# greysun/GraphEmbeddings

Measured on AMD Instinct MI355X. Metric: scored triples/sec/GPU (d=200), higher is better.
Workload: dtype f32

## Files before the change

graphembeddings_amd/build.py:

```python
from __future__ import annotations

import os
import shutil
import subprocess
import sys

HERE = os.path.dirname(os.path.abspath(__file__))
CSRC = os.path.join(HERE, "csrc")
LIB = os.path.join(HERE, "libge_hip.so")
SOURCES = ["ge_capi.hip", "ge_complex.hip", "ge_rows.hip", "ge_hole.hip", "ge_1vk.hip", "ge_train.hip", "ge_prep_big.hip", "ge_shard.hip", "ge_spectral.hip", "ge_rank.hip", "ge_rank_pipe.hip", "ge_rank_f16.hip", "ge_known.hip", "ge_transx.hip", "ge_transr.hip", "ge_transx_rank.hip", "ge_neighbors.hip", "ge_transx_relrank.hip", "ge_classify.hip"]
HEADERS = ["ge_common.h", "ge_launch.h", "ge_step_id.h", "ge_prep.h", "ge_complex_dev.h", "ge_rank_dev.h", "ge_sweep_route.h", "ge_trans.h", "ge_trans_dev.h", "ge_f16_dev.h", "ge_topk_dev.h", "ge_bernoulli_dev.h", os.path.join("..", "..", "include", "ge_hip.h")]
ARCH = "gfx950"


def _hipcc() -> str:
    for cand in (os.environ.get("HIPCC"), shutil.which("hipcc"), "/opt/rocm/bin/hipcc"):
        if cand and os.path.exists(cand):
            return cand
    raise RuntimeError("hipcc not found: libge_hip.so cannot be built (ROCm toolchain required)")


def needs_build() -> bool:
    if not os.path.exists(LIB):
        return True
    t = os.path.getmtime(LIB)
    deps = [os.path.join(CSRC, s) for s in SOURCES + HEADERS] + [os.path.abspath(__file__)]
    return any(os.path.getmtime(p) > t for p in deps)


FILE_FLAGS = {"ge_hole.hip": ["-fno-slp-vectorize"]}
OBJDIR = os.path.join(HERE, "_obj")


def build(force: bool = False, verbose: bool = False, extra_flags=()) -> str:
    if not force and not needs_build():
        return LIB
    os.makedirs(OBJDIR, exist_ok=True)
    cc = _hipcc()
    common = ["-O3", f"--offload-arch={ARCH}", "-std=c++17", "-fPIC", "-Wall", "-Wno-unused-function", *extra_flags,
              *os.environ.get("GE_CXXFLAGS", "").split()]
    procs = []
    for src in SOURCES:
        obj = os.path.join(OBJDIR, src.replace(".hip", ".o"))
        cmd = [cc, *common, *FILE_FLAGS.get(src, []), "-c", src, "-o", obj]
# ... 19 lines not shown
```

graphembeddings_amd/csrc/ge_complex.hip:

```cpp
#include "ge_complex_dev.h"
#include "ge_launch.h"

namespace ge {

template <bool SPEC, int VEC, int LPT, int NITER>
__global__ __launch_bounds__(kBlock) void complex_score_kernel(
    const float* __restrict__ table, int64_t N, int d, const int32_t* __restrict__ triples, int64_t B,
    float max_norm, int apply_sigmoid, float* __restrict__ out, float label, float l2,
    const float* __restrict__ table_sumsq, int64_t ld) {
  constexpr int GPW = kWave / LPT;
  const int lane = threadIdx.x & (kWave - 1), sub = lane % LPT, grp = lane / LPT;
  const int64_t wave = ((int64_t)blockIdx.x * blockDim.x + threadIdx.x) >> 6;
  const int64_t nwaves = ((int64_t)gridDim.x * blockDim.x) >> 6;
  const int k = d >> 1, nvec = k / VEC;
  const float wscale = 1.0f / (float)d;
  for (int64_t base = wave * GPW; base < B; base += nwaves * GPW) {
    const int64_t g = base + grp;
    const bool live = g < B;
    int32_t hi = 0, ti = 0, ri = 0;
    if (live) { hi = triples[3 * g]; ti = triples[3 * g + 1]; ri = triples[3 * g + 2]; }
    const bool bad = bad3(N, hi, ti, ri);
    if (bad) { hi = ti = ri = 0; }
    Row<VEC, NITER> h, t, r;
    load_row_at<VEC, LPT, NITER>(table + (int64_t)hi * ld, k, nvec, sub, h);
// ... 138 lines not shown
        store_vec<VEC>(gp + k + j * VEC, pim_);
      }
    }
  }
}


template <int CTRL>
__device__ __forceinline__ float dpp_add(float v) {
  return v + __int_as_float(__builtin_amdgcn_update_dpp(0, __float_as_int(v), CTRL, 0xF, 0xF, false));
}
template <int LPT>
__device__ __forceinline__ float group_sum_dpp(float v) {
  static_assert(LPT == 16 || LPT == 32 || LPT == 64, "lane group");
  v = dpp_add<0xB1>(v);
  v = dpp_add<0x4E>(v);
  v = dpp_add<0x141>(v);
  v = dpp_add<0x140>(v);
  if (LPT >= 32) v += __int_as_float(__builtin_amdgcn_ds_swizzle(__float_as_int(v), 0x401F));
  if (LPT >= 64) v += __shfl_xor(v, 32, kWave);
  return v;
}

template <int VEC, int LPT, int NITER>
__device__ __forceinline__ void load_row_clamped(const float* __restrict__ p, int k, int nvec, int sub, Row<VEC, NITER>& R) {
#pragma unroll
  for (int it = 0; it < NITER; ++it) {
    const int j = min(sub + it * LPT, nvec - 1);
    load_vec<VEC>(p + j * VEC, R.re[it]);
    load_vec<VEC>(p + k + j * VEC, R.im[it]);
  }
}

template <bool SPEC, bool SHARD, bool ORD, int VEC, int LPT, int NITER, bool PEER = false>
__global__ __launch_bounds__(kBlock, (VEC * NITER <= 4 ? 4 : 2)) void complex_hinge_grad_plan_kernel(
    const float* rows, int64_t N, int d, const int32_t* __restrict__ pos,
    const int32_t* __restrict__ neg, int64_t B, float margin, float lr, float max_norm,
    float* __restrict__ loss, int32_t* __restrict__ grad_idx, float* __restrict__ grad_val,
    const int32_t* __restrict__ slot_item, float* table_rw, ShardGrad sg, const int32_t* __restrict__ order) {
  constexpr int kSlotDirect = -2;
  constexpr int GPW = kWave / LPT;
  const int lane = threadIdx.x & (kWave - 1), sub = lane % LPT, grp = lane / LPT;
  const int wave = (int)(((int64_t)blockIdx.x * blockDim.x + threadIdx.x) >> 6);
  const int nwaves = (int)(((int64_t)gridDim.x * blockDim.x) >> 6);
  const int nB = (int)B;
  const int k = d >> 1, nvec = k / VEC;
  const float wscale = 1.0f / (float)d;
  const float neg_lr = -lr;
  float act[NITER];
#pragma unroll
  for (int it = 0; it < NITER; ++it) act[it] = (sub + it * LPT < nvec) ? 1.f : 0.f;
  const int per = ORD ? ((nB + nwaves - 1) / nwaves + GPW - 1) / GPW * GPW : 0;
  float racc_re[NITER][VEC], racc_im[NITER][VEC];
#pragma unroll
  for (int it = 0; it < NITER; ++it)
#pragma unroll
    for (int v = 0; v < VEC; ++v) { racc_re[it][v] = 0.f; racc_im[it][v] = 0.f; }
  int32_t cur_rel = -1;
  int cur_slot = -1;
  auto flush = [&]() {
    float* o = grad_val + (int64_t)cur_slot * d;
#pragma unroll
    for (int it = 0; it < NITER; ++it) {
      const int j = sub + it * LPT;
      if (j < nvec) {
        store_vec<VEC>(o + j * VEC, racc_re[it]);
        store_vec<VEC>(o + k + j * VEC, racc_im[it]);
      }
#pragma unroll
      for (int v = 0; v < VEC; ++v) { racc_re[it][v] = 0.f; racc_im[it][v] = 0.f; }
    }
    if (sub == 0) grad_idx[cur_slot] = cur_rel;
// ... 81 lines not shown
      }
      accP += act[it] * tP; accN += act[it] * tN;
    }
    {
      auto ssq = [&](const Row<VEC, NITER>& R) {
        float s = 0.f;
#pragma unroll
        for (int it = 0; it < NITER; ++it) {
          float t = 0.f;
#pragma unroll
          for (int v = 0; v < VEC; ++v) {
            const float q = R.re[it][v] * R.re[it][v] + R.im[it][v] * R.im[it][v];
            if (SPEC) t += (it == 0 && v == 0 && first_el) ? q : 2.f * q;
            else t += q;
          }
          s += act[it] * t;
        }
        return s;
      };
      qF = ssq(xF); qV = ssq(xV); qC = ssq(xC); qR = ssq(xR);
    }
    float ssF = group_sum_dpp<LPT>(qF), ssV = group_sum_dpp<LPT>(qV);
    float ssC = group_sum_dpp<LPT>(qC), ssR = group_sum_dpp<LPT>(qR);
    float srP = group_sum_dpp<LPT>(accP), srN = group_sum_dpp<LPT>(accN);
    if (SPEC) { ssF *= wscale; ssV *= wscale; ssC *= wscale; ssR *= wscale; srP *= wscale; srN *= wscale; }
    float invF, invV, invC, invR;
    const float scF = clip_scale(ssF, max_norm, invF), scV = clip_scale(ssV, max_norm, invV);
    const float scC = clip_scale(ssC, max_norm, invC), scR = clip_scale(ssR, max_norm, invR);
    const float sigP = sigmoidf_dev(srP * (hs ? scV : scF) * (hs ? scF : scV) * scR);
    const float sigN = sigmoidf_dev(srN * (hs ? scC : scF) * (hs ? scF : scC) * scR);
    const float pre = sigP - sigN + margin;
    const bool on = live && !bad && (pre >= 0.f);
    if (live && sub == 0) loss[g] = bad ? __builtin_nanf("") : fmaxf(pre, 0.f);
    const bool same = c == idV;
    const int slot0 = g * 6;
    const int32_t tagF = hs ? tag[1] : tag[0], tagV = hs ? tag[0] : tag[1], tagR = tag[2], tagC = hs ? tag[3] : tag[4];
    const bool dirF = slot_item && live && tagF == kSlotDirect, dirV = slot_item && live && tagV == kSlotDirect;
    const bool dirR = slot_item && live && tagR == kSlotDirect, dirC = slot_item && live && !same && tagC == kSlotDirect;
    const bool sndF = SHARD && slot_item && live && tagF <= -3, sndV = SHARD && slot_item && live && tagV <= -3;
    const bool sndR = SHARD && slot_item && live && tagR <= -3, sndC = SHARD && slot_item && live && !same && tagC <= -3;
    const bool accum = ORD && !dirR && !sndR;
    if (accum && live && cur_slot >= 0 && p2 != cur_rel) flush();
    if (live && sub == 0) {
      const int32_t giF = (on && !dirF && !sndF) ? idF : -1, giV = (on && !dirV && !sndV) ? idV : -1;
      const int32_t giC = (on && !same && !dirC && !sndC) ? c : -1;
      grad_idx[slot0] = hs ? giV : giF;
      grad_idx[slot0 + 1] = hs ? giF : giV;
      grad_idx[slot0 + 2] = (on && !dirR && !sndR && !accum) ? p2 : -1;
      grad_idx[slot0 + 3] = hs ? giC : -1;
      grad_idx[slot0 + 4] = hs ? -1 : giC;
      grad_idx[slot0 + 5] = -1;
    }
    if (!on) {
      if (SHARD && (sndF || sndV || sndR || sndC)) {
        float z[VEC];
#pragma unroll
        for (int v = 0; v < VEC; ++v) z[v] = 0.f;
        auto zero_row = [&](bool doit, int32_t tg) {
          if (!doit) return;
          float* o = sg.gsum + (int64_t)(-3 - tg) * d;
#pragma unroll
          for (int it = 0; it < NITER; ++it) {
            const int j = sub + it * LPT;
            if (j < nvec) { store_vec<VEC>(o + j * VEC, z); store_vec<VEC>(o + k + j * VEC, z); }
          }
        };
// ... 347 lines not shown
  Shape s;
  if (ld <= 0) ld = d;
  if (ld < d) return GE_EINVAL;
  if (!pick_shape(d, table, 2, s, ld)) return (d <= 0 || (d & 1)) ? GE_EINVAL : GE_ENOTSUP;
  if (B == 0) return 0;
  const int gpb = (kBlock / kWave) * (kWave / s.lpt);
  const int grid = grid_for(B, gpb);
#define CALL(V, L, NI) \
  hipLaunchKernelGGL((complex_score_kernel<SP, V, L, NI>), dim3(grid), dim3(kBlock), 0, st, table, N, d, triples, B, max_norm, apply_sigmoid, out, label, l2, table_sumsq, ld)
  GE_DISPATCH_SPEC(spectral, s, CALL);
#undef CALL
  return launch_status();
}

int complex_hinge_loss_launch(const float* table, int64_t N, int32_t d, const int32_t* pos,
                              const int32_t* neg, int64_t B, float margin, float max_norm, float* loss,
                              float* sig_out, hipStream_t st, int spectral) {
  Shape s;
  if (!pick_shape(d, table, 2, s)) return (d <= 0 || (d & 1)) ? GE_EINVAL : GE_ENOTSUP;
  if (B == 0) return 0;
  const int gpb = (kBlock / kWave) * (kWave / s.lpt);
  const int grid = grid_for(B, gpb);
#define CALL(V, L, NI) \
  hipLaunchKernelGGL((complex_hinge_loss_kernel<SP, V, L, NI>), dim3(grid), dim3(kBlock), 0, st, table, N, d, pos, neg, B, margin, max_norm, loss, sig_out)
  GE_DISPATCH_SPEC(spectral, s, CALL);
#undef CALL
  return launch_status();
}

int complex_hinge_grad_launch(const float* rows, int64_t N, int32_t d, const int32_t* pos,
                              const int32_t* neg, int64_t B, float margin, float lr, float max_norm,
                              float* loss, int32_t* grad_idx, float* grad_val, hipStream_t st,
                              hipEvent_t ev_start, hipEvent_t ev_stop, const int32_t* slot_item, float* table_rw,
                              int spectral, const int32_t* order) {
  Shape s;
  if (!pick_shape(d, rows, 2, s)) return (d <= 0 || (d & 1)) ? GE_EINVAL : GE_ENOTSUP;
  while (s.vec > 1 && (reinterpret_cast<uintptr_t>(grad_val) % (s.vec * 4)) != 0) return GE_EINVAL;
  if ((slot_item != nullptr) != (table_rw != nullptr)) return GE_EINVAL;
  if (B == 0) return 0;
  const int gpb = (kBlock / kWave) * (kWave / s.lpt);
  const int grid = grid_for(B, gpb);
#define CALL(V, L, NI) \
  hipExtLaunchKernelGGL((complex_hinge_grad_kernel<SP, V, L, NI>), dim3(grid), dim3(kBlock), 0, st, ev_start, ev_stop, 0, rows, N, d, pos, neg, B, margin, lr, max_norm, loss, grad_idx, grad_val, slot_item, table_rw)
#define CALLO(V, L, NI) \
  hipExtLaunchKernelGGL((complex_hinge_grad_plan_kernel<SP, false, true, V, L, NI>), dim3(grid), dim3(kBlock), 0, st, ev_start, ev_stop, 0, rows, N, d, pos, neg, B, margin, lr, max_norm, loss, grad_idx, grad_val, slot_item, table_rw, ShardGrad{}, order)
#define CALLP(V, L, NI) \
  hipExtLaunchKernelGGL((complex_hinge_grad_plan_kernel<SP, false, false, V, L, NI>), dim3(grid), dim3(kBlock), 0, st, ev_start, ev_stop, 0, rows, N, d, pos, neg, B, margin, lr, max_norm, loss, grad_idx, grad_val, slot_item, table_rw, ShardGrad{}, nullptr)
  if (order) { GE_DISPATCH_SPEC(spectral, s, CALLO); }
  else if (slot_item) { GE_DISPATCH_SPEC(spectral, s, CALLP); }
  else { GE_DISPATCH_SPEC(spectral, s, CALL); }
#undef CALLP
#undef CALLO
#undef CALL
  return launch_status();
}

int shard_hinge_grad_launch(float* shard, int32_t d, const float* staged, const int32_t* pos_src, const int32_t* neg_src,
                            const int32_t* slot_item, int32_t R, int64_t B, float margin, float lr, float max_norm,
                            float* loss, int32_t* grad_idx, float* grad_val, float* gsum, int spectral, hipStream_t st,
                            hipEvent_t ev_start, hipEvent_t ev_stop, const int32_t* order, const float* const* peers, int n_peers) {
  Shape s;
  if (!pick_shape(d, shard, 2, s)) return (d <= 0 || (d & 1)) ? GE_EINVAL : GE_ENOTSUP;
  for (const void* q : {(const void*)grad_val, (const void*)staged, (const void*)gsum})
    if (q && (reinterpret_cast<uintptr_t>(q) % (s.vec * 4)) != 0) return GE_EINVAL;
  if (B == 0) return 0;
  const int gpb = (kBlock / kWave) * (kWave / s.lpt);
  const int grid = grid_for(B, gpb);
  ShardGrad sg{staged, R, pos_src, neg_src, gsum, {}};
  if (peers) {
    if (staged || n_peers > kMaxPeers) return GE_EINVAL;
    for (int i = 0; i < kMaxPeers; ++i) sg.peer[i] = i < n_peers ? peers[i] : nullptr;
  }
#define CALL(V, L, NI) \
  hipExtLaunchKernelGGL((complex_hinge_grad_plan_kernel<SP, true, ORDF, V, L, NI, PEERF>), dim3(grid), dim3(kBlock), 0, st, ev_start, ev_stop, 0, shard, (int64_t)R, d, nullptr, nullptr, B, margin, lr, max_norm, loss, grad_idx, grad_val, slot_item, shard, sg, order)
  if (peers) {
    constexpr bool PEERF = true;
    if (order) { constexpr bool ORDF = true; GE_DISPATCH_SPEC(spectral, s, CALL); }
    else { constexpr bool ORDF = false; GE_DISPATCH_SPEC(spectral, s, CALL); }
  } else {
    constexpr bool PEERF = false;
    if (order) { constexpr bool ORDF = true; GE_DISPATCH_SPEC(spectral, s, CALL); }
    else { constexpr bool ORDF = false; GE_DISPATCH_SPEC(spectral, s, CALL); }
  }
#undef CALL
  return launch_status();
}

int complex_logloss_grad_launch(const float* rows, int64_t N, int32_t d, const int32_t* triples,
                                const float* labels, int64_t M, float lr, float max_norm, float l2,
                                const float* table_sumsq, float* loss, int32_t* grad_idx, float* grad_val,
                                hipStream_t st, const int32_t* negs, int64_t B, float row_scale, float neg_lr_eff,
                                hipEvent_t ev_start, hipEvent_t ev_stop) {
  Shape s;
  if (!pick_shape(d, rows, 2, s)) return (d <= 0 || (d & 1)) ? GE_EINVAL : GE_ENOTSUP;
  if ((reinterpret_cast<uintptr_t>(grad_val) % (s.vec * 4)) != 0) return GE_EINVAL;
  if (M == 0) return 0;
  if (!negs) neg_lr_eff = -lr;
  const int gpb = (kBlock / kWave) * (kWave / s.lpt);
  const int grid = grid_for(M, gpb);
#define CALL(V, L, NI) \
  hipExtLaunchKernelGGL((complex_logloss_grad_kernel<V, L, NI>), dim3(grid), dim3(kBlock), 0, st, ev_start, ev_stop, 0, rows, N, d, triples, labels, negs, B, M, neg_lr_eff, max_norm, l2, row_scale, table_sumsq, loss, grad_idx, grad_val)
  GE_DISPATCH_SHAPE(s, 2, CALL);
#undef CALL
  return launch_status();
}

int table_sumsq_launch(const float* table, int64_t n, float* out, hipStream_t st) {
// ... 17 lines not shown
```

graphembeddings_amd/csrc/ge_launch.h:

```cpp
#pragma once
#include <assert.h>
#include <hip/hip_runtime.h>
#include <stddef.h>
#include <stdint.h>

#include "ge_step_id.h"
#include "ge_sweep_route.h"
#include "ge_trans.h"

namespace ge {

struct TileGeom;
struct ShardOut;

int complex_max_dim();
int complex_score_launch(const float* table, int64_t N, int32_t d, const int32_t* triples, int64_t B, float max_norm,
                         int apply_sigmoid, float* out, hipStream_t st, int spectral = 0, float label = 0.f, float l2 = 0.f,
                         const float* table_sumsq = nullptr, int64_t ld = 0);
int complex_hinge_loss_launch(const float* table, int64_t N, int32_t d, const int32_t* pos, const int32_t* neg, int64_t B,
                              float margin, float max_norm, float* loss, float* sig_out, hipStream_t st, int spectral = 0);
int complex_hinge_grad_launch(const float* rows, int64_t N, int32_t d, const int32_t* pos, const int32_t* neg, int64_t B,
                              float margin, float lr, float max_norm, float* loss, int32_t* grad_idx, float* grad_val,
                              hipStream_t st, hipEvent_t ev_start = nullptr, hipEvent_t ev_stop = nullptr,
                              const int32_t* slot_item = nullptr, float* table_rw = nullptr, int spectral = 0,
                              const int32_t* order = nullptr);
int complex_logloss_grad_launch(const float* rows, int64_t N, int32_t d, const int32_t* triples, const float* labels,
                                int64_t M, float lr, float max_norm, float l2, const float* table_sumsq, float* loss,
                                int32_t* grad_idx, float* grad_val, hipStream_t st, const int32_t* negs = nullptr,
                                int64_t B = 0, float row_scale = 1.f, float neg_lr_eff = 0.f, hipEvent_t ev_start = nullptr,
                                hipEvent_t ev_stop = nullptr);
int shard_hinge_grad_launch(float* shard, int32_t d, const float* staged, const int32_t* pos_src, const int32_t* neg_src,
                            const int32_t* slot_item, int32_t R, int64_t B, float margin, float lr, float max_norm,
                            float* loss, int32_t* grad_idx, float* grad_val, float* gsum, int spectral, hipStream_t st,
                            hipEvent_t ev_start, hipEvent_t ev_stop, const int32_t* order, const float* const* peers,
                            int n_peers);
int table_sumsq_launch(const float* table, int64_t n, float* out, hipStream_t st);
int table_scale_launch(float* table, int64_t n, float factor, hipStream_t st);

int hole_score_launch(const float* table, int64_t N, int32_t d, const int32_t* triples, int64_t B, float max_norm,
                      int apply_sigmoid, float* out, hipStream_t st);
int hole_hinge_loss_launch(const float* table, int64_t N, int32_t d, const int32_t* pos, const int32_t* neg, int64_t B,
                           float margin, float max_norm, float* loss, float* sig_out, hipStream_t st);
int hole_hinge_grad_launch(const float* rows, int64_t N, int32_t d, const int32_t* pos, const int32_t* neg, int64_t B,
                           float margin, float lr, float max_norm, float* loss, int32_t* grad_idx, float* grad_val,
                           hipStream_t st, hipEvent_t ev_start = nullptr, hipEvent_t ev_stop = nullptr);

int hole_spectral_launch(float* table, int64_t N, int32_t d, int inverse, hipStream_t st);

int scatter_add_rows_launch(float* table, int64_t N, int32_t d, const int32_t* idx, const float* val, int64_t R,
                            hipStream_t st, hipEvent_t ev_start = nullptr, hipEvent_t ev_stop = nullptr);
int gather_rows_launch(const float* table, int64_t N, int32_t d, const int32_t* idx, int64_t R, float* out, hipStream_t st);
int corrupt_batch_launch(const int32_t* pos, int64_t B, const TypeSampler& ts, uint64_t step, int32_t* neg, hipStream_t st);
struct SamplerArgs {
  const int32_t* triples; int64_t T; const int64_t* bh_key; const int32_t* bh_ent; const int64_t* bt_key;
  const int32_t* bt_ent; int64_t n_known; const uint32_t* tail_threshold; int32_t n_rel, n_ent;
};
int bernoulli_corrupt_launch(const int32_t* pos, int64_t B, const SamplerArgs& s, int32_t ent_lo, uint64_t seed,
                             uint64_t step, int32_t* neg, hipStream_t st);
// ... 166 lines not shown
```

graphembeddings_amd/csrc/ge_train.hip:

```cpp
#include "ge_prep.h"
#include "ge_launch.h"
#include <algorithm>
#include <cmath>
#include <utility>

namespace ge {

__global__ __launch_bounds__(kPrepThreads) void train_prepare_kernel(
    const int32_t* __restrict__ triples, int64_t T, int64_t first_row, int64_t B, int64_t s0,
    const int32_t* __restrict__ id_to_type, int64_t N, const int64_t* __restrict__ type_offsets,
    int32_t n_types, const int32_t* __restrict__ type_ids, uint64_t seed, uint64_t global_step0,
    int32_t padded_size, int32_t mode, int direct, int n_pass, int bits, int negs, int32_t* __restrict__ prep) {
  extern __shared__ __attribute__((aligned(16))) unsigned long long keys[];
  const PrepLayout L = prep_layout(B, negs);
  const int P = (int)L.P, R = P / kPrepThreads;
  unsigned* hist = reinterpret_cast<unsigned*>(keys + P);
  int* wtot = reinterpret_cast<int*>(hist + kPrepWaves * kMaxRadix);
  const int tid = threadIdx.x, lane = tid & (kWave - 1), wave = tid >> 6;
  const int sub = blockIdx.y;
  const int64_t s = s0 + blockIdx.x;
  const int32_t* pos = triples + 3 * step_row(first_row, T, B, s);
  int32_t* rec = prep + (int64_t)blockIdx.x * L.stride;
  int32_t* neg = rec;
  int32_t* slot_item = rec + L.off_slot;
  int32_t* subrec = rec + L.off_sub + sub * L.sub_stride;
  int32_t* items = subrec + L.off_items;
  int32_t* islots = subrec + L.off_islots;
  const int64_t i0 = (int64_t)sub * kSub;
  const int S = (int)((L.units - i0) < kSub ? (L.units - i0) : kSub);
  const uint64_t step = global_step0 + (uint64_t)s;
  const bool batch_heads = (mode == GE_CORRUPT_BATCH_COIN) ? batch_coin_heads(seed, step) : false;
  constexpr unsigned long long kInvalid = ~0ull;

  if (direct)
// ... 600 lines not shown
static TrainWs train_ws(void* base, int64_t B, int32_t d) {
  const HingeWs g = hinge_ws(base, B, d);
  const size_t region = grad_region_bytes(B, d);
  const int ring = grad_ring(B, d);
  const size_t grad = g.bytes + (size_t)(ring - 1) * region;
  return TrainWs{g, ring, region / sizeof(float), ws_at<int32_t>(base, grad), grad + prep_region_bytes(B, 0)};
}
template <class Need, class Step>
static size_t largest_need_up_to(int64_t B, Need need, Step step) {
  size_t best = need(B);
  int64_t b = 1;
  while (b < B) {
    const auto v = step(b);
    if (step(B) == v) break;
    int64_t lo = b, hi = B;
    while (hi - lo > 1) { const int64_t mid = lo + (hi - lo) / 2; if (step(mid) == v) lo = mid; else hi = mid; }
    best = std::max(best, need(lo));
    b = hi;
  }
  return best;
}

size_t train_ws_bytes(int64_t B, int32_t d) {
  if (!train_fast_ok(B, d)) return hinge_ws(nullptr, B, d).bytes;
  return largest_need_up_to(B, [&](int64_t b) { return train_ws(nullptr, b, d).bytes; },
                            [&](int64_t b) { return std::make_pair(prep_chunk_steps(b), (int64_t)grad_ring(b, d)); });
}

static size_t prep_lds_bytes(const PrepLayout& L) {
  return sizeof(unsigned long long) * (size_t)L.P + sizeof(unsigned) * kPrepWaves * kMaxRadix + sizeof(int) * 32;
}

static int prepare_launch(const StepSeq& q, int64_t s0, int64_t n, const TypeSampler& ts, int direct, int32_t* out,
                          void* scratch, hipStream_t st, int negs = 0) {
  const PrepLayout L = prep_layout(q.B, negs);
  if (L.n_sub > 1)
    return prepare_big_launch(q, s0, n, ts, direct, out, scratch, st, negs);
  const SortBits sb = sort_bits_for(ts.N);
  const int n_pass = sb.n_pass, bits = sb.bits;
  const size_t lds = prep_lds_bytes(L);
  hipError_t e = hipFuncSetAttribute(reinterpret_cast<const void*>(train_prepare_kernel),
                                     hipFuncAttributeMaxDynamicSharedMemorySize, 160 * 1024);
  if (e != hipSuccess) return (int)e;
  hipLaunchKernelGGL(train_prepare_kernel, dim3((unsigned)n, (unsigned)L.n_sub), dim3(kPrepThreads), lds, st, q.triples,
                     q.T, q.first_row, q.B, s0, ts.id_to_type, ts.N, ts.type_offsets, ts.n_types, ts.type_ids, ts.seed,
                     q.global_step0, ts.padded_size, ts.mode, direct, n_pass, bits, negs, out);
  return launch_status();
}

#define GE_HIP_TRY(expr) do { hipError_t e_ = (expr); if (e_ != hipSuccess) return (int)e_; } while (0)

struct Pipeline {
  int device = -1;
  hipStream_t side = nullptr;
  hipEvent_t prep_done[2] = {nullptr, nullptr};
  hipEvent_t buf_free[2] = {nullptr, nullptr};
  bool live = false;
  StepIdentity id = {};
  int64_t next_abs = 0, resident[2] = {-1, -1};
};

int pipeline_create(void** out) {
  Pipeline* p = new Pipeline();
  hipError_t e = hipGetDevice(&p->device);
  if (e == hipSuccess) e = hipStreamCreateWithFlags(&p->side, hipStreamNonBlocking);
  for (int i = 0; i < 2 && e == hipSuccess; ++i) {
    e = hipEventCreateWithFlags(&p->prep_done[i], hipEventDisableTiming);
    if (e == hipSuccess) e = hipEventCreateWithFlags(&p->buf_free[i], hipEventDisableTiming);
  }
  if (e != hipSuccess) { delete p; return (int)e; }
  *out = p;
  return 0;
}
int pipeline_reset(void* h) {
  if (!h) return GE_EINVAL;
  static_cast<Pipeline*>(h)->live = false;
  return 0;
}
int pipeline_destroy(void* h) {
  if (!h) return GE_EINVAL;
  Pipeline* p = static_cast<Pipeline*>(h);
  if (p->side) { (void)hipStreamSynchronize(p->side); (void)hipStreamDestroy(p->side); }
  for (int i = 0; i < 2; ++i) {
    if (p->prep_done[i]) (void)hipEventDestroy(p->prep_done[i]);
    if (p->buf_free[i]) (void)hipEventDestroy(p->buf_free[i]);
  }
  delete p;
  return 0;
}

static inline int64_t norm_row(int64_t first_row, int64_t T, int64_t B) {
  int64_t f = first_row % T;
  if (f + B > T) f = 0;
  return f;
}
static inline bool continues(const StepSeq& a, int64_t done, const StepSeq& b) {
  return b.global_step0 == a.global_step0 + (uint64_t)done &&
         norm_row(b.first_row, b.T, b.B) == step_row(a.first_row, b.T, b.B, done);
}

class PrepCursor {
 public:
  PrepCursor(const StepIdentity& id, Pipeline* handle, int32_t* prep_base, hipStream_t st)
      : id_(id), L_(prep_layout(id.seq.B, id.negs)), K_(prep_chunk_steps(id.seq.B, id.negs)),
        buf_ints_((int64_t)(prep_chunk_bytes(id.seq.B, id.negs) / sizeof(int32_t))), base_(prep_base), st_(st),
        pipe_(handle ? handle : &local_), own_side_(handle != nullptr) {
    id_.seq.first_row = norm_row(id.seq.first_row, id.seq.T, id.seq.B);
  }

  int begin() {
    if (own_side_) {
      int dev = -1;
      GE_HIP_TRY(hipGetDevice(&dev));
      if (dev != pipe_->device) return GE_EINVAL;
      Pipeline* p = pipe_;
      const bool cont = p->live && same_source(p->id, id_) && continues(p->id.seq, p->next_abs, id_.seq);
      if (!cont) {
        p->live = true;
        p->id = id_;
        p->next_abs = 0;
        p->resident[0] = p->resident[1] = -1;
      }
      base_abs_ = p->next_abs;
    } else {
      pipe_->id = id_;
      pipe_->side = st_;
    }
    return 0;
  }

  int step(int64_t s, const int32_t** rec) {
    const int64_t abs_s = base_abs_ + s, chunk = abs_s / K_, in_chunk = abs_s % K_;
    if (s == 0 || in_chunk == 0) {
      int rc = ensure(chunk);
      if (rc) return rc;
      if (own_side_) {
        rc = ensure(chunk + 1);
        if (rc) return rc;
        GE_HIP_TRY(hipStreamWaitEvent(st_, pipe_->prep_done[chunk & 1], 0));
      }
    }
    *rec = base_ + (chunk & 1) * buf_ints_ + in_chunk * L_.stride;
    return 0;
  }

  int finish(int64_t n_steps, const int32_t** last_rec) {
    const int64_t la = base_abs_ + n_steps - 1;
    *last_rec = base_ + ((la / K_) & 1) * buf_ints_ + (la % K_) * L_.stride;
    if (own_side_) {
      GE_HIP_TRY(hipStreamWaitEvent(st_, pipe_->prep_done[((la / K_) + 1) & 1], 0));
      pipe_->next_abs = base_abs_ + n_steps;
    }
    return 0;
  }

  const PrepLayout& layout() const { return L_; }

 private:
  int ensure(int64_t c) {
    const int b = (int)(c & 1);
    if (pipe_->resident[b] == c) return 0;
    if (own_side_) {
      GE_HIP_TRY(hipEventRecord(pipe_->buf_free[b], st_));
      GE_HIP_TRY(hipStreamWaitEvent(pipe_->side, pipe_->buf_free[b], 0));
    }
    int rc = prepare_launch(pipe_->id.seq, c * K_, K_, id_.ts, id_.direct, base_ + b * buf_ints_, base_ + 2 * buf_ints_,
                            pipe_->side, id_.negs);
    if (rc) return rc;
    if (own_side_) GE_HIP_TRY(hipEventRecord(pipe_->prep_done[b], pipe_->side));
    pipe_->resident[b] = c;
    return 0;
  }

  StepIdentity id_;
  PrepLayout L_;
  int64_t K_, buf_ints_;
  int32_t* base_;
  hipStream_t st_;
  Pipeline local_;
  Pipeline* pipe_;
  bool own_side_;
  int64_t base_abs_ = 0;
};

int train_steps_run(float* table, int32_t d, const StepSeq& q, int64_t n_steps, const TypeSampler& ts, float margin,
                    const StepHyper& hp, int model, float* loss, int keep_all_losses, int32_t* neg_ws, void* workspace,
                    size_t workspace_bytes, void** ev_pairs, int ev_kernel, void* pipe_handle, hipStream_t st) {
  const int64_t N = ts.N, B = q.B;
  const float max_norm = hp.max_norm;
  if (n_steps <= 0) return 0;
  const int deterministic = (model & GE_STEP_DETERMINISTIC) ? 1 : 0;
  model &= ~GE_STEP_DETERMINISTIC;
  const bool transform = model == GE_MODEL_HOLE && !(d & 1);
  const bool spectral = transform || model == GE_MODEL_HOLE_SPECTRAL;
  const bool hole_direct = (model == GE_MODEL_HOLE && (d & 1)) || model == GE_MODEL_HOLE_DIRECT;
  if (transform) { int rc = hole_spectral_launch(table, N, d, 0, st); if (rc) return rc; }
  const bool fast = train_fast_ok(B, d) && workspace_bytes >= train_ws_bytes(B, d);
  const TrainWs w = fast ? train_ws(workspace, B, d) : TrainWs{hinge_ws(workspace, B, d), 1, 0, nullptr, 0};
  int32_t* const gidx = w.g.gidx;
  float* const gval0 = w.g.gval;
  const int ring = w.ring;
  const size_t region_floats = w.region_floats;
  const int direct = hole_direct ? 0 : 1;
  PrepCursor cur(StepIdentity{q, ts, d, direct, 0, workspace}, fast ? static_cast<Pipeline*>(pipe_handle) : nullptr, w.prep, st);
  const PrepLayout& L = cur.layout();
  if (fast) { int rc = cur.begin(); if (rc) return rc; }
  for (int64_t s = 0; s < n_steps; ++s) {
    const uint64_t gs = q.global_step0 + (uint64_t)s;
    const float lr = hp.lr_at(gs);
    const int32_t* pos = q.triples + 3 * step_row(q.first_row, q.T, B, s);
    float* loss_s = keep_all_losses ? loss + s * B : loss;
    hipEvent_t e0 = ev_pairs ? (hipEvent_t)ev_pairs[2 * s] : nullptr;
    hipEvent_t e1 = ev_pairs ? (hipEvent_t)ev_pairs[2 * s + 1] : nullptr;
    int rc;
    const int32_t* neg;
    const int32_t* step_rec = nullptr;
    if (e0 && ev_kernel == 0) (void)hipEventRecord(e0, st);
    if (fast) {
      rc = cur.step(s, &step_rec);
      if (rc) return rc;
      neg = step_rec;
    } else {
      rc = corrupt_batch_launch(pos, B, ts, gs, neg_ws, st);
      if (rc) return rc;
      neg = neg_ws;
    }
    if (e1 && ev_kernel == 0) (void)hipEventRecord(e1, st);
    float* gval = gval0 + (size_t)(gs % (uint64_t)ring) * region_floats;
    hipEvent_t g0 = ev_kernel == 1 ? e0 : nullptr, g1 = ev_kernel == 1 ? e1 : nullptr;
    hipEvent_t a0 = ev_kernel == 2 ? e0 : nullptr, a1 = ev_kernel == 2 ? e1 : nullptr;
    const bool dir = fast && direct;
    rc = hole_direct ? hole_hinge_grad_launch(table, N, d, pos, neg, B, margin, lr, max_norm, loss_s, gidx, gval, st, g0, g1)
                     : complex_hinge_grad_launch(table, N, d, pos, neg, B, margin, lr, max_norm, loss_s, gidx, gval, st, g0, g1,
                                                 dir ? step_rec + L.off_slot : nullptr, dir ? table : nullptr, spectral ? 1 : 0,
                                                 (fast && L.off_order >= 0) ? step_rec + L.off_order : nullptr);
    if (rc) return rc;
    if (fast) rc = apply_sorted_launch(table, d, L, step_rec, gidx, gval, st, a0, a1, deterministic);
    else rc = scatter_add_rows_launch(table, N, d, gidx, gval, 6 * B, st, a0, a1);
    if (rc) return rc;
  }
  if (fast) {
    const int32_t* last = nullptr;
    int rc = cur.finish(n_steps, &last);
    if (rc) return rc;
    GE_HIP_TRY(hipMemcpyAsync(neg_ws, last, sizeof(int32_t) * 3 * (size_t)B, hipMemcpyDeviceToDevice, st));
  }
  if (transform) { int rc = hole_spectral_launch(table, N, d, 1, st); if (rc) return rc; }
  return 0;
}

static size_t logloss_region_bytes(int64_t M, int32_t d) { return align_up(sizeof(float) * 3 * (size_t)M * (size_t)d, 256); }
LoglossWs logloss_ws(void* base, int64_t M, int32_t d) {
  const size_t idx = align_up(sizeof(int32_t) * 3 * (size_t)M, 256);
  return LoglossWs{ws_at<float>(base, 0), ws_at<int32_t>(base, 256), ws_at<float>(base, 256 + idx),
                   256 + idx + logloss_region_bytes(M, d)};
}
static size_t logloss_ring(int64_t B, int32_t negs, int32_t d) {
  size_t ring = ((size_t)64 << 20) / logloss_region_bytes((int64_t)(1 + negs) * B, d) + 1;
  if (ring < 2) ring = 2;
  if (ring > 8) ring = 8;
  return ring;
}
struct LoglossLoopWs { LoglossWs g; size_t ring, region; int32_t* prep; size_t bytes; };
static LoglossLoopWs train_logloss_ws(void* base, int64_t B, int32_t negs, int32_t d) {
  const int64_t M = (int64_t)(1 + negs) * B;
  const LoglossWs g = logloss_ws(base, M, d);
  const size_t region = logloss_region_bytes(M, d), ring = logloss_ring(B, negs, d);
  const size_t grad = g.bytes + (ring - 1) * region;
  return LoglossLoopWs{g, ring, region, ws_at<int32_t>(base, grad), grad + prep_region_bytes(B, negs)};
}
size_t train_logloss_ws_bytes(int64_t B, int32_t negs, int32_t d) {
  return largest_need_up_to(B, [&](int64_t b) { return train_logloss_ws(nullptr, b, negs, d).bytes; },
                            [&](int64_t b) { return std::make_pair(prep_chunk_steps(b, negs), (int64_t)logloss_ring(b, negs, d)); });
}

int train_logloss_run(float* table, int32_t d, const StepSeq& q, int64_t n_steps, const TypeSampler& ts, int32_t negs,
                      float l2, const StepHyper& hp, float* loss, int keep_all_losses, int32_t* neg_ws, void* workspace,
                      size_t workspace_bytes, void* pipe_handle, hipStream_t st) {
  const int64_t N = ts.N, B = q.B;
  const float max_norm = hp.max_norm;
  if (n_steps <= 0) return 0;
  if (workspace_bytes < train_logloss_ws_bytes(B, negs, d)) return GE_ENOMEM;
  const size_t M = (size_t)(1 + negs) * (size_t)B;
  const LoglossLoopWs w = train_logloss_ws(workspace, B, negs, d);
  float* const sumsq = w.g.sumsq;
  int32_t* const gidx = w.g.gidx;
  char* const gval0 = reinterpret_cast<char*>(w.g.gval);
  const size_t ring = w.ring, region = w.region;
  PrepCursor cur(StepIdentity{q, ts, d, 0, negs, workspace}, static_cast<Pipeline*>(pipe_handle), w.prep, st);
  const PrepLayout& L = cur.layout();
  int rc = cur.begin();
  if (rc) return rc;
  double g = 1.0;
  auto materialise = [&]() -> int {
    if (g == 1.0) return 0;
    int r2 = table_scale_launch(table, N * (int64_t)d, (float)g, st);
    g = 1.0;
    return r2;
  };
  for (int64_t s = 0; s < n_steps; ++s) {
    const uint64_t gs = q.global_step0 + (uint64_t)s;
    const float lr = hp.lr_at(gs);
    const int32_t* pos = q.triples + 3 * step_row(q.first_row, q.T, B, s);
    const int32_t* step_rec = nullptr;
    rc = cur.step(s, &step_rec);
    if (rc) return rc;
    const double f = 1.0 - (double)lr * (double)M * (double)l2;
    double g_new = g * f;
    if (g_new == 0.0 || std::fabs(g_new) < 9.1e-13 || std::fabs(g_new) > 1.1e12) {
      rc = materialise();
      if (rc) return rc;
      g_new = 1.0;
    }
    const bool want_loss = keep_all_losses || s == n_steps - 1;
    if (want_loss) { rc = table_sumsq_launch(table, N * (int64_t)d, sumsq, st); if (rc) return rc; }
    float* loss_s = keep_all_losses ? loss + s * (int64_t)M : loss;
    float* gval = reinterpret_cast<float*>(gval0 + (size_t)(gs % (uint64_t)ring) * region);
    const bool dense_now = (g_new == 1.0 && g * f != 1.0);
    const float neg_lr_eff = (float)(-(double)lr / (dense_now ? 1.0 : g_new));
    rc = complex_logloss_grad_launch(table, N, d, pos, nullptr, (int64_t)M, lr, max_norm, l2, want_loss ? sumsq : nullptr,
                                     loss_s, gidx, gval, st, step_rec, B, (float)g, neg_lr_eff, nullptr, nullptr);
    if (rc) return rc;
    if (dense_now) {
      rc = table_scale_launch(table, N * (int64_t)d, (float)f, st);
      if (rc) return rc;
    }
    rc = apply_sorted_launch(table, d, L, step_rec, gidx, gval, st, nullptr, nullptr);
    if (rc) return rc;
    g = g_new;
  }
  rc = materialise();
  if (rc) return rc;
  const int32_t* last = nullptr;
  rc = cur.finish(n_steps, &last);
  if (rc) return rc;
  GE_HIP_TRY(hipMemcpyAsync(neg_ws, last, sizeof(int32_t) * 3 * (size_t)negs * (size_t)B, hipMemcpyDeviceToDevice, st));
  return 0;
}

static size_t prepared_records_bytes(int64_t B, int64_t n_steps) {
  return align_up(sizeof(int32_t) * (size_t)n_steps * (size_t)prep_layout(B).stride, 256);
}
size_t train_prepare_bytes(int64_t B, int64_t n_steps) {
  return prepared_records_bytes(B, n_steps) + prep_big_scratch_bytes(B, 0, n_steps);
}
int train_prepare_run(const StepSeq& q, int64_t n_steps, const TypeSampler& ts, int direct, int32_t* out, hipStream_t st) {
  if (n_steps == 0) return 0;
  StepSeq from = q;
  from.first_row = norm_row(q.first_row, q.T, q.B);
  return prepare_launch(from, 0, n_steps, ts, direct ? 1 : 0, out, ws_at<void>(out, prepared_records_bytes(q.B, n_steps)), st);
}

void train_prepared_layout(int64_t B, int64_t* out) {
  const PrepLayout L = prep_layout(B);
  out[0] = L.stride; out[1] = L.n_sub; out[2] = L.S; out[3] = L.off_slot; out[4] = L.off_sub;
  out[5] = L.sub_stride; out[6] = L.off_items; out[7] = L.off_islots;
}

}
```

Baseline: 592.1 million.

## Restructure prep-chunk lookahead, cache workspace sizing, emit negatives from kernel

Moves the double-buffered negative-sample preparation schedule into a LookaheadState planner. The next chunk's prep is now launched after the current step's kernels rather than before, and stream waits are issued only when a buffer is actually unordered relative to the caller stream. It also caches the shared-memory attribute call and workspace-size computation per pipeline. The last step's negatives are written directly by the hinge kernel instead of through a trailing device-to-device memcpy. This cuts host API overhead and avoids redundant waits, at the cost of more complex cross-call state that could misorder buffers if the planner is wrong.

```diff
diff --git a/graphembeddings_amd/build.py b/graphembeddings_amd/build.py
--- a/graphembeddings_amd/build.py
+++ b/graphembeddings_amd/build.py
@@ -9,7 +9,7 @@
 CSRC = os.path.join(HERE, "csrc")
 LIB = os.path.join(HERE, "libge_hip.so")
 SOURCES = ["ge_capi.hip", "ge_complex.hip", "ge_rows.hip", "ge_hole.hip", "ge_1vk.hip", "ge_train.hip", "ge_prep_big.hip", "ge_shard.hip", "ge_spectral.hip", "ge_rank.hip", "ge_rank_pipe.hip", "ge_rank_f16.hip", "ge_known.hip", "ge_transx.hip", "ge_transr.hip", "ge_transx_rank.hip", "ge_neighbors.hip", "ge_transx_relrank.hip", "ge_classify.hip"]
-HEADERS = ["ge_common.h", "ge_launch.h", "ge_step_id.h", "ge_prep.h", "ge_complex_dev.h", "ge_rank_dev.h", "ge_sweep_route.h", "ge_trans.h", "ge_trans_dev.h", "ge_f16_dev.h", "ge_topk_dev.h", "ge_bernoulli_dev.h", os.path.join("..", "..", "include", "ge_hip.h")]
+HEADERS = ["ge_common.h", "ge_launch.h", "ge_step_id.h", "ge_lookahead.h", "ge_prep.h", "ge_complex_dev.h", "ge_rank_dev.h", "ge_sweep_route.h", "ge_trans.h", "ge_trans_dev.h", "ge_f16_dev.h", "ge_topk_dev.h", "ge_bernoulli_dev.h", os.path.join("..", "..", "include", "ge_hip.h")]
 ARCH = "gfx950"
 
 
diff --git a/graphembeddings_amd/csrc/ge_complex.hip b/graphembeddings_amd/csrc/ge_complex.hip
--- a/graphembeddings_amd/csrc/ge_complex.hip
+++ b/graphembeddings_amd/csrc/ge_complex.hip
@@ -194,12 +194,13 @@
   }
 }
 
-template <bool SPEC, bool SHARD, bool ORD, int VEC, int LPT, int NITER, bool PEER = false>
+template <bool SPEC, bool SHARD, bool ORD, int VEC, int LPT, int NITER, bool PEER = false, bool NEGOUT = false>
 __global__ __launch_bounds__(kBlock, (VEC * NITER <= 4 ? 4 : 2)) void complex_hinge_grad_plan_kernel(
     const float* rows, int64_t N, int d, const int32_t* __restrict__ pos,
     const int32_t* __restrict__ neg, int64_t B, float margin, float lr, float max_norm,
     float* __restrict__ loss, int32_t* __restrict__ grad_idx, float* __restrict__ grad_val,
-    const int32_t* __restrict__ slot_item, float* table_rw, ShardGrad sg, const int32_t* __restrict__ order) {
+    const int32_t* __restrict__ slot_item, float* table_rw, ShardGrad sg, const int32_t* __restrict__ order,
+    int32_t* __restrict__ neg_out) {
   constexpr int kSlotDirect = -2;
   constexpr int GPW = kWave / LPT;
   const int lane = threadIdx.x & (kWave - 1), sub = lane % LPT, grp = lane / LPT;
@@ -347,6 +348,9 @@
     const float pre = sigP - sigN + margin;
     const bool on = live && !bad && (pre >= 0.f);
     if (live && sub == 0) loss[g] = bad ? __builtin_nanf("") : fmaxf(pre, 0.f);
+    if constexpr (NEGOUT && !SHARD) {
+      if (live && sub == 0) { neg_out[3 * g] = raw[3]; neg_out[3 * g + 1] = raw[4]; neg_out[3 * g + 2] = raw[2]; }
+    }
     const bool same = c == idV;
     const int slot0 = g * 6;
     const int32_t tagF = hs ? tag[1] : tag[0], tagV = hs ? tag[0] : tag[1], tagR = tag[2], tagC = hs ? tag[3] : tag[4];
@@ -760,23 +764,32 @@
                               const int32_t* neg, int64_t B, float margin, float lr, float max_norm,
                               float* loss, int32_t* grad_idx, float* grad_val, hipStream_t st,
                               hipEvent_t ev_start, hipEvent_t ev_stop, const int32_t* slot_item, float* table_rw,
-                              int spectral, const int32_t* order) {
+                              int spectral, const int32_t* order, int32_t* neg_out) {
   Shape s;
   if (!pick_shape(d, rows, 2, s)) return (d <= 0 || (d & 1)) ? GE_EINVAL : GE_ENOTSUP;
   while (s.vec > 1 && (reinterpret_cast<uintptr_t>(grad_val) % (s.vec * 4)) != 0) return GE_EINVAL;
   if ((slot_item != nullptr) != (table_rw != nullptr)) return GE_EINVAL;
+  if (neg_out && !slot_item) return GE_EINVAL;
   if (B == 0) return 0;
   const int gpb = (kBlock / kWave) * (kWave / s.lpt);
   const int grid = grid_for(B, gpb);
 #define CALL(V, L, NI) \
   hipExtLaunchKernelGGL((complex_hinge_grad_kernel<SP, V, L, NI>), dim3(grid), dim3(kBlock), 0, st, ev_start, ev_stop, 0, rows, N, d, pos, neg, B, margin, lr, max_norm, loss, grad_idx, grad_val, slot_item, table_rw)
 #define CALLO(V, L, NI) \
-  hipExtLaunchKernelGGL((complex_hinge_grad_plan_kernel<SP, false, true, V, L, NI>), dim3(grid), dim3(kBlock), 0, st, ev_start, ev_stop, 0, rows, N, d, pos, neg, B, margin, lr, max_norm, loss, grad_idx, grad_val, slot_item, table_rw, ShardGrad{}, order)
+  hipExtLaunchKernelGGL((complex_hinge_grad_plan_kernel<SP, false, true, V, L, NI>), dim3(grid), dim3(kBlock), 0, st, ev_start, ev_stop, 0, rows, N, d, pos, neg, B, margin, lr, max_norm, loss, grad_idx, grad_val, slot_item, table_rw, ShardGrad{}, order, nullptr)
 #define CALLP(V, L, NI) \
-  hipExtLaunchKernelGGL((complex_hinge_grad_plan_kernel<SP, false, false, V, L, NI>), dim3(grid), dim3(kBlock), 0, st, ev_start, ev_stop, 0, rows, N, d, pos, neg, B, margin, lr, max_norm, loss, grad_idx, grad_val, slot_item, table_rw, ShardGrad{}, nullptr)
-  if (order) { GE_DISPATCH_SPEC(spectral, s, CALLO); }
+  hipExtLaunchKernelGGL((complex_hinge_grad_plan_kernel<SP, false, false, V, L, NI>), dim3(grid), dim3(kBlock), 0, st, ev_start, ev_stop, 0, rows, N, d, pos, neg, B, margin, lr, max_norm, loss, grad_idx, grad_val, slot_item, table_rw, ShardGrad{}, nullptr, nullptr)
+#define CALLON(V, L, NI) \
+  hipExtLaunchKernelGGL((complex_hinge_grad_plan_kernel<SP, false, true, V, L, NI, false, true>), dim3(grid), dim3(kBlock), 0, st, ev_start, ev_stop, 0, rows, N, d, pos, neg, B, margin, lr, max_norm, loss, grad_idx, grad_val, slot_item, table_rw, ShardGrad{}, order, neg_out)
+#define CALLPN(V, L, NI) \
+  hipExtLaunchKernelGGL((complex_hinge_grad_plan_kernel<SP, false, false, V, L, NI, false, true>), dim3(grid), dim3(kBlock), 0, st, ev_start, ev_stop, 0, rows, N, d, pos, neg, B, margin, lr, max_norm, loss, grad_idx, grad_val, slot_item, table_rw, ShardGrad{}, nullptr, neg_out)
+  if (neg_out && order) { GE_DISPATCH_SPEC(spectral, s, CALLON); }
+  else if (neg_out) { GE_DISPATCH_SPEC(spectral, s, CALLPN); }
+  else if (order) { GE_DISPATCH_SPEC(spectral, s, CALLO); }
   else if (slot_item) { GE_DISPATCH_SPEC(spectral, s, CALLP); }
   else { GE_DISPATCH_SPEC(spectral, s, CALL); }
+#undef CALLPN
+#undef CALLON
 #undef CALLP
 #undef CALLO
 #undef CALL
@@ -800,7 +813,7 @@
     for (int i = 0; i < kMaxPeers; ++i) sg.peer[i] = i < n_peers ? peers[i] : nullptr;
   }
 #define CALL(V, L, NI) \
-  hipExtLaunchKernelGGL((complex_hinge_grad_plan_kernel<SP, true, ORDF, V, L, NI, PEERF>), dim3(grid), dim3(kBlock), 0, st, ev_start, ev_stop, 0, shard, (int64_t)R, d, nullptr, nullptr, B, margin, lr, max_norm, loss, grad_idx, grad_val, slot_item, shard, sg, order)
+  hipExtLaunchKernelGGL((complex_hinge_grad_plan_kernel<SP, true, ORDF, V, L, NI, PEERF>), dim3(grid), dim3(kBlock), 0, st, ev_start, ev_stop, 0, shard, (int64_t)R, d, nullptr, nullptr, B, margin, lr, max_norm, loss, grad_idx, grad_val, slot_item, shard, sg, order, nullptr)
   if (peers) {
     constexpr bool PEERF = true;
     if (order) { constexpr bool ORDF = true; GE_DISPATCH_SPEC(spectral, s, CALL); }
diff --git a/graphembeddings_amd/csrc/ge_launch.h b/graphembeddings_amd/csrc/ge_launch.h
--- a/graphembeddings_amd/csrc/ge_launch.h
+++ b/graphembeddings_amd/csrc/ge_launch.h
@@ -23,7 +23,7 @@
                               float margin, float lr, float max_norm, float* loss, int32_t* grad_idx, float* grad_val,
                               hipStream_t st, hipEvent_t ev_start = nullptr, hipEvent_t ev_stop = nullptr,
                               const int32_t* slot_item = nullptr, float* table_rw = nullptr, int spectral = 0,
-                              const int32_t* order = nullptr);
+                              const int32_t* order = nullptr, int32_t* neg_out = nullptr);
 int complex_logloss_grad_launch(const float* rows, int64_t N, int32_t d, const int32_t* triples, const float* labels,
                                 int64_t M, float lr, float max_norm, float l2, const float* table_sumsq, float* loss,
                                 int32_t* grad_idx, float* grad_val, hipStream_t st, const int32_t* negs = nullptr,
diff --git a/graphembeddings_amd/csrc/ge_lookahead.h b/graphembeddings_amd/csrc/ge_lookahead.h
--- /dev/null
+++ b/graphembeddings_amd/csrc/ge_lookahead.h
@@ -0,0 +1,50 @@
+#pragma once
+#include <stdint.h>
+
+namespace ge {
+
+inline int64_t lookahead_cover(int64_t K) { return (K + 3) / 4; }
+
+struct LookaheadState {
+  int64_t resident[2] = {-1, -1};
+  bool ordered[2] = {true, true};
+  void forget() { resident[0] = resident[1] = -1; ordered[0] = ordered[1] = true; }
+  void new_stream() { for (int b = 0; b < 2; ++b) ordered[b] = resident[b] < 0; }
+};
+
+struct LookaheadStep {
+  int64_t chunk, in_chunk;
+  int buf;
+  int64_t prepare_before;
+  bool wait_before;
+  int64_t prepare_after;
+};
+
+inline LookaheadStep lookahead_step(LookaheadState& st, int64_t K, int64_t abs_s, int64_t s, int64_t n_steps, bool side) {
+  LookaheadStep p{abs_s / K, abs_s % K, (int)((abs_s / K) & 1), -1, false, -1};
+  if (s != 0 && p.in_chunk != 0) return p;
+  if (st.resident[p.buf] != p.chunk) {
+    p.prepare_before = p.chunk;
+    st.resident[p.buf] = p.chunk;
+    st.ordered[p.buf] = !side;
+  }
+  if (!st.ordered[p.buf]) {
+    p.wait_before = true;
+    st.ordered[p.buf] = true;
+  }
+  if (side && st.resident[p.buf ^ 1] != p.chunk + 1 && (s == 0 || n_steps - s >= lookahead_cover(K))) {
+    p.prepare_after = p.chunk + 1;
+    st.resident[p.buf ^ 1] = p.chunk + 1;
+    st.ordered[p.buf ^ 1] = false;
+  }
+  return p;
+}
+
+inline int lookahead_end(LookaheadState& st) {
+  int mask = 0;
+  for (int b = 0; b < 2; ++b)
+    if (!st.ordered[b]) { mask |= 1 << b; st.ordered[b] = true; }
+  return mask;
+}
+
+}
diff --git a/graphembeddings_amd/csrc/ge_train.hip b/graphembeddings_amd/csrc/ge_train.hip
--- a/graphembeddings_amd/csrc/ge_train.hip
+++ b/graphembeddings_amd/csrc/ge_train.hip
@@ -1,5 +1,6 @@
 #include "ge_prep.h"
 #include "ge_launch.h"
+#include "ge_lookahead.h"
 #include <algorithm>
 #include <cmath>
 #include <utility>
@@ -666,16 +667,19 @@
 }
 
 static int prepare_launch(const StepSeq& q, int64_t s0, int64_t n, const TypeSampler& ts, int direct, int32_t* out,
-                          void* scratch, hipStream_t st, int negs = 0) {
+                          void* scratch, hipStream_t st, int negs = 0, bool* lds_set = nullptr) {
   const PrepLayout L = prep_layout(q.B, negs);
   if (L.n_sub > 1)
     return prepare_big_launch(q, s0, n, ts, direct, out, scratch, st, negs);
   const SortBits sb = sort_bits_for(ts.N);
   const int n_pass = sb.n_pass, bits = sb.bits;
   const size_t lds = prep_lds_bytes(L);
-  hipError_t e = hipFuncSetAttribute(reinterpret_cast<const void*>(train_prepare_kernel),
-                                     hipFuncAttributeMaxDynamicSharedMemorySize, 160 * 1024);
-  if (e != hipSuccess) return (int)e;
+  if (!lds_set || !*lds_set) {
+    hipError_t e = hipFuncSetAttribute(reinterpret_cast<const void*>(train_prepare_kernel),
+                                       hipFuncAttributeMaxDynamicSharedMemorySize, 160 * 1024);
+    if (e != hipSuccess) return (int)e;
+    if (lds_set) *lds_set = true;
+  }
   hipLaunchKernelGGL(train_prepare_kernel, dim3((unsigned)n, (unsigned)L.n_sub), dim3(kPrepThreads), lds, st, q.triples,
                      q.T, q.first_row, q.B, s0, ts.id_to_type, ts.N, ts.type_offsets, ts.n_types, ts.type_ids, ts.seed,
                      q.global_step0, ts.padded_size, ts.mode, direct, n_pass, bits, negs, out);
@@ -691,8 +695,21 @@
   hipEvent_t buf_free[2] = {nullptr, nullptr};
   bool live = false;
   StepIdentity id = {};
-  int64_t next_abs = 0, resident[2] = {-1, -1};
+  int64_t next_abs = 0;
+  LookaheadState look;
+  hipStream_t caller = nullptr;
+  bool have_caller = false;
+  bool prep_lds_set = false;
+  int64_t need_B = -1;
+  int32_t need_negs = 0, need_d = 0;
+  size_t need_bytes = 0;
 };
+static size_t ws_need(Pipeline* p, int64_t B, int32_t negs, int32_t d) {
+  if (p && p->need_B == B && p->need_negs == negs && p->need_d == d) return p->need_bytes;
+  const size_t need = negs > 0 ? train_logloss_ws_bytes(B, negs, d) : train_ws_bytes(B, d);
+  if (p) { p->need_B = B; p->need_negs = negs; p->need_d = d; p->need_bytes = need; }
+  return need;
+}
 
 int pipeline_create(void** out) {
   Pipeline* p = new Pipeline();
@@ -735,10 +752,10 @@
 
 class PrepCursor {
  public:
-  PrepCursor(const StepIdentity& id, Pipeline* handle, int32_t* prep_base, hipStream_t st)
+  PrepCursor(const StepIdentity& id, Pipeline* handle, int32_t* prep_base, hipStream_t st, int64_t n_steps)
       : id_(id), L_(prep_layout(id.seq.B, id.negs)), K_(prep_chunk_steps(id.seq.B, id.negs)),
         buf_ints_((int64_t)(prep_chunk_bytes(id.seq.B, id.negs) / sizeof(int32_t))), base_(prep_base), st_(st),
-        pipe_(handle ? handle : &local_), own_side_(handle != nullptr) {
+        pipe_(handle ? handle : &local_), own_side_(handle != nullptr), n_steps_(n_steps) {
     id_.seq.first_row = norm_row(id.seq.first_row, id.seq.T, id.seq.B);
   }
 
@@ -753,7 +770,12 @@
         p->live = true;
         p->id = id_;
         p->next_abs = 0;
-        p->resident[0] = p->resident[1] = -1;
+        p->look.forget();
+      }
+      if (!p->have_caller || p->caller != st_) {
+        p->look.new_stream();
+        p->caller = st_;
+        p->have_caller = true;
       }
       base_abs_ = p->next_abs;
     } else {
@@ -764,26 +786,30 @@
   }
 
   int step(int64_t s, const int32_t** rec) {
-    const int64_t abs_s = base_abs_ + s, chunk = abs_s / K_, in_chunk = abs_s % K_;
-    if (s == 0 || in_chunk == 0) {
-      int rc = ensure(chunk);
+    plan_ = lookahead_step(pipe_->look, K_, base_abs_ + s, s, n_steps_, own_side_);
+    if (plan_.prepare_before >= 0) {
+      int rc = launch(plan_.prepare_before);
       if (rc) return rc;
-      if (own_side_) {
-        rc = ensure(chunk + 1);
-        if (rc) return rc;
-        GE_HIP_TRY(hipStreamWaitEvent(st_, pipe_->prep_done[chunk & 1], 0));
-      }
-    }
-    *rec = base_ + (chunk & 1) * buf_ints_ + in_chunk * L_.stride;
+    }
+    if (plan_.wait_before) GE_HIP_TRY(hipStreamWaitEvent(st_, pipe_->prep_done[plan_.buf], 0));
+    *rec = base_ + plan_.buf * buf_ints_ + plan_.in_chunk * L_.stride;
     return 0;
   }
 
-  int finish(int64_t n_steps, const int32_t** last_rec) {
-    const int64_t la = base_abs_ + n_steps - 1;
+  int after_step() {
+    const int64_t c = plan_.prepare_after;
+    plan_.prepare_after = -1;
+    return c >= 0 ? launch(c) : 0;
+  }
+
+  int finish(const int32_t** last_rec) {
+    const int64_t la = base_abs_ + n_steps_ - 1;
     *last_rec = base_ + ((la / K_) & 1) * buf_ints_ + (la % K_) * L_.stride;
     if (own_side_) {
-      GE_HIP_TRY(hipStreamWaitEvent(st_, pipe_->prep_done[((la / K_) + 1) & 1], 0));
-      pipe_->next_abs = base_abs_ + n_steps;
+      const int mask = lookahead_end(pipe_->look);
+      for (int b = 0; b < 2; ++b)
+        if (mask >> b & 1) GE_HIP_TRY(hipStreamWaitEvent(st_, pipe_->prep_done[b], 0));
+      pipe_->next_abs = base_abs_ + n_steps_;
     }
     return 0;
   }
@@ -791,18 +817,21 @@
   const PrepLayout& layout() const { return L_; }
 
  private:
-  int ensure(int64_t c) {
+  int launch(int64_t c) {
+    const int rc = launch_checked(c);
+    if (rc && own_side_) pipe_->live = false;
+    return rc;
+  }
+  int launch_checked(int64_t c) {
     const int b = (int)(c & 1);
-    if (pipe_->resident[b] == c) return 0;
     if (own_side_) {
       GE_HIP_TRY(hipEventRecord(pipe_->buf_free[b], st_));
       GE_HIP_TRY(hipStreamWaitEvent(pipe_->side, pipe_->buf_free[b], 0));
     }
     int rc = prepare_launch(pipe_->id.seq, c * K_, K_, id_.ts, id_.direct, base_ + b * buf_ints_, base_ + 2 * buf_ints_,
-                            pipe_->side, id_.negs);
+                            pipe_->side, id_.negs, &pipe_->prep_lds_set);
     if (rc) return rc;
     if (own_side_) GE_HIP_TRY(hipEventRecord(pipe_->prep_done[b], pipe_->side));
-    pipe_->resident[b] = c;
     return 0;
   }
 
@@ -814,7 +843,9 @@
   Pipeline local_;
   Pipeline* pipe_;
   bool own_side_;
+  int64_t n_steps_;
   int64_t base_abs_ = 0;
+  LookaheadStep plan_ = {0, 0, 0, -1, false, -1};
 };
 
 int train_steps_run(float* table, int32_t d, const StepSeq& q, int64_t n_steps, const TypeSampler& ts, float margin,
@@ -829,16 +860,18 @@
   const bool spectral = transform || model == GE_MODEL_HOLE_SPECTRAL;
   const bool hole_direct = (model == GE_MODEL_HOLE && (d & 1)) || model == GE_MODEL_HOLE_DIRECT;
   if (transform) { int rc = hole_spectral_launch(table, N, d, 0, st); if (rc) return rc; }
-  const bool fast = train_fast_ok(B, d) && workspace_bytes >= train_ws_bytes(B, d);
+  const bool fast = train_fast_ok(B, d) && workspace_bytes >= ws_need(static_cast<Pipeline*>(pipe_handle), B, 0, d);
   const TrainWs w = fast ? train_ws(workspace, B, d) : TrainWs{hinge_ws(workspace, B, d), 1, 0, nullptr, 0};
   int32_t* const gidx = w.g.gidx;
   float* const gval0 = w.g.gval;
   const int ring = w.ring;
   const size_t region_floats = w.region_floats;
   const int direct = hole_direct ? 0 : 1;
-  PrepCursor cur(StepIdentity{q, ts, d, direct, 0, workspace}, fast ? static_cast<Pipeline*>(pipe_handle) : nullptr, w.prep, st);
+  PrepCursor cur(StepIdentity{q, ts, d, direct, 0, workspace}, fast ? static_cast<Pipeline*>(pipe_handle) : nullptr, w.prep, st,
+                 n_steps);
   const PrepLayout& L = cur.layout();
   if (fast) { int rc = cur.begin(); if (rc) return rc; }
+  const bool neg_by_kernel = fast && !hole_direct;
   for (int64_t s = 0; s < n_steps; ++s) {
     const uint64_t gs = q.global_step0 + (uint64_t)s;
     const float lr = hp.lr_at(gs);
@@ -867,17 +900,20 @@
     rc = hole_direct ? hole_hinge_grad_launch(table, N, d, pos, neg, B, margin, lr, max_norm, loss_s, gidx, gval, st, g0, g1)
                      : complex_hinge_grad_launch(table, N, d, pos, neg, B, margin, lr, max_norm, loss_s, gidx, gval, st, g0, g1,
                                                  dir ? step_rec + L.off_slot : nullptr, dir ? table : nullptr, spectral ? 1 : 0,
-                                                 (fast && L.off_order >= 0) ? step_rec + L.off_order : nullptr);
+                                                 (fast && L.off_order >= 0) ? step_rec + L.off_order : nullptr,
+                                                 (neg_by_kernel && s == n_steps - 1) ? neg_ws : nullptr);
     if (rc) return rc;
     if (fast) rc = apply_sorted_launch(table, d, L, step_rec, gidx, gval, st, a0, a1, deterministic);
     else rc = scatter_add_rows_launch(table, N, d, gidx, gval, 6 * B, st, a0, a1);
     if (rc) return rc;
+    if (fast) { rc = cur.after_step(); if (rc) return rc; }
   }
   if (fast) {
     const int32_t* last = nullptr;
-    int rc = cur.finish(n_steps, &last);
+    int rc = cur.finish(&last);
     if (rc) return rc;
-    GE_HIP_TRY(hipMemcpyAsync(neg_ws, last, sizeof(int32_t) * 3 * (size_t)B, hipMemcpyDeviceToDevice, st));
+    if (!neg_by_kernel)
+      GE_HIP_TRY(hipMemcpyAsync(neg_ws, last, sizeof(int32_t) * 3 * (size_t)B, hipMemcpyDeviceToDevice, st));
   }
   if (transform) { int rc = hole_spectral_launch(table, N, d, 1, st); if (rc) return rc; }
   return 0;
@@ -914,14 +950,14 @@
   const int64_t N = ts.N, B = q.B;
   const float max_norm = hp.max_norm;
   if (n_steps <= 0) return 0;
-  if (workspace_bytes < train_logloss_ws_bytes(B, negs, d)) return GE_ENOMEM;
+  if (workspace_bytes < ws_need(static_cast<Pipeline*>(pipe_handle), B, negs, d)) return GE_ENOMEM;
   const size_t M = (size_t)(1 + negs) * (size_t)B;
   const LoglossLoopWs w = train_logloss_ws(workspace, B, negs, d);
   float* const sumsq = w.g.sumsq;
   int32_t* const gidx = w.g.gidx;
   char* const gval0 = reinterpret_cast<char*>(w.g.gval);
   const size_t ring = w.ring, region = w.region;
-  PrepCursor cur(StepIdentity{q, ts, d, 0, negs, workspace}, static_cast<Pipeline*>(pipe_handle), w.prep, st);
+  PrepCursor cur(StepIdentity{q, ts, d, 0, negs, workspace}, static_cast<Pipeline*>(pipe_handle), w.prep, st, n_steps);
   const PrepLayout& L = cur.layout();
   int rc = cur.begin();
   if (rc) return rc;
@@ -961,12 +997,14 @@
     }
     rc = apply_sorted_launch(table, d, L, step_rec, gidx, gval, st, nullptr, nullptr);
     if (rc) return rc;
+    rc = cur.after_step();
+    if (rc) return rc;
     g = g_new;
   }
   rc = materialise();
   if (rc) return rc;
   const int32_t* last = nullptr;
-  rc = cur.finish(n_steps, &last);
+  rc = cur.finish(&last);
   if (rc) return rc;
   GE_HIP_TRY(hipMemcpyAsync(neg_ws, last, sizeof(int32_t) * 3 * (size_t)negs * (size_t)B, hipMemcpyDeviceToDevice, st));
   return 0;
```

Result: no change. 589.0 million (-0.5%).
